# jfdev001/algebraic-multigrid

Measured on AMD Instinct MI355X. Metric: V-cycles/sec, 2D Poisson N=4096^2 (fine-grid smoother HBM GB/s under roofline), higher is better.
Workload: dtype f64; 1 GPU; 2D 5-point Poisson 4096x4096 (Grid::laplacian/rhs), true Jacobi smoother omega=0.6 2+2 sweeps, 16-level V-cycle, coarsest 511 dofs, fp64, 1xMI355X; smoother has no counterpart in the reference: pinned to the oracle twin; n=4096, dim=2, levels=16, smoother=jacobi, sweeps=2, graph=True, coarse_solve=band-chain (LDS-resident scalar recurrence, half-bandwidth <= 3, bit-exact), layout=dict

## Files before the change

algebraic-multigrid_amd/csrc/kernels.hip:

```cpp
#include <hip/hip_runtime.h>
#include <cstdlib>
#include <stdint.h>

#include <cstdio>
#include <type_traits>
#include <utility>
#include <vector>
#include <algorithm>
#include <cmath>

#include "kernels.hpp"

namespace amg_hip {

__device__ __forceinline__ void lds_barrier() {
  asm volatile("s_waitcnt lgkmcnt(0)\n\ts_barrier" ::: "memory");
}

constexpr bool mode_cheb(int m) { return (m & ~3) == 16; }
constexpr bool mode_jac(int m) { return m == CSR_JACOBI || mode_cheb(m); }
constexpr bool cheb_first(int m) { return (m & 1) != 0; }
constexpr bool cheb_last(int m) { return (m & 2) != 0; }
template <int MODE>
__device__ __forceinline__ double cheb_update(double t, double xi, double di, double alpha, double beta,
// ... 4612 lines not shown
                     omega, C, ring - 1);
  return hipGetLastError();
}
hipError_t launch_gs_scan(int64_t n, const DictRef& D, const double* b, double* u, double* s_old,
                          bool backward, int mode, double omega, int C, int ring, hipStream_t st) {
  if (n <= 0) return hipSuccess;
  if (!dict_args_ok(n, D.words, D.wmax, D.ntab) || C < 1 || C > GS_SCAN_MAX_CHUNK || ring < 2 || ring > 16384 ||
      (ring & (ring - 1)) || !s_old)
    return hipErrorInvalidValue;
  hipError_t r = hipSuccess;
  (void)dict_dispatch_wu(D.words, D.wmax, [&](auto W, auto U) {
    r = launch_gs_scan_wu<decltype(W)::value, decltype(U)::value>(n, D, b, u, s_old, backward ? 1 : 0,
                                                                  mode, omega, C, ring, st);
  });
  return r;
}

__device__ __forceinline__ bool spin_until_one(uint32_t* w, uint32_t* timeout) {
  const unsigned long long t0 = wall_clock64();
  while (__hip_atomic_load(w, __ATOMIC_ACQUIRE, __HIP_MEMORY_SCOPE_SYSTEM) != 1u) {
    if (wall_clock64() - t0 > 200000000ull) {
      __hip_atomic_store(timeout, 1u, __ATOMIC_RELAXED, __HIP_MEMORY_SCOPE_SYSTEM);
      return false;
    }
    __builtin_amdgcn_s_sleep(8);
  }
  __hip_atomic_store(w, 0u, __ATOMIC_RELAXED, __HIP_MEMORY_SCOPE_SYSTEM);
  return true;
}

__global__ __launch_bounds__(256) void halo_exchange_kernel(HaloArgs a) {
  const int t = threadIdx.x;
  if (t == 0) {
    if (a.cnt_prev > 0) spin_until_one(a.my_free_from_prev, a.timeout);
    if (a.cnt_next > 0) spin_until_one(a.my_free_from_next, a.timeout);
  }
  __syncthreads();
  for (int64_t i = t; i < a.cnt_prev; i += 256)
    __builtin_nontemporal_store(a.src_prev[i], a.dst_prev + i);
  for (int64_t i = t; i < a.cnt_next; i += 256)
    __builtin_nontemporal_store(a.src_next[i], a.dst_next + i);
  __threadfence_system();
  __syncthreads();
  if (t == 0) {
    if (a.cnt_prev > 0)
      __hip_atomic_store(a.data_at_prev, 1u, __ATOMIC_RELEASE, __HIP_MEMORY_SCOPE_SYSTEM);
    if (a.cnt_next > 0)
      __hip_atomic_store(a.data_at_next, 1u, __ATOMIC_RELEASE, __HIP_MEMORY_SCOPE_SYSTEM);
    if (a.recv_prev) spin_until_one(a.my_data_from_prev, a.timeout);
    if (a.recv_next) spin_until_one(a.my_data_from_next, a.timeout);
    __threadfence_system();
  }
}
__global__ void halo_ack_kernel(uint32_t* free_at_prev, uint32_t* free_at_next) {
  if (threadIdx.x == 0) {
    if (free_at_prev) __hip_atomic_store(free_at_prev, 1u, __ATOMIC_RELEASE, __HIP_MEMORY_SCOPE_SYSTEM);
    if (free_at_next) __hip_atomic_store(free_at_next, 1u, __ATOMIC_RELEASE, __HIP_MEMORY_SCOPE_SYSTEM);
  }
}
__global__ void halo_wait_free_kernel(HaloArgs a) {
  if (threadIdx.x == 0) {
    if (a.cnt_prev > 0) spin_until_one(a.my_free_from_prev, a.timeout);
    if (a.cnt_next > 0) spin_until_one(a.my_free_from_next, a.timeout);
  }
}
__global__ __launch_bounds__(256) void halo_copy_kernel(HaloArgs a) {
  const int64_t t = (int64_t)blockIdx.x * 256 + threadIdx.x, nt = (int64_t)gridDim.x * 256;
  for (int64_t i = t; i < a.cnt_prev; i += nt) __builtin_nontemporal_store(a.src_prev[i], a.dst_prev + i);
  for (int64_t i = t; i < a.cnt_next; i += nt) __builtin_nontemporal_store(a.src_next[i], a.dst_next + i);
  __threadfence_system();
}
__global__ void halo_publish_wait_kernel(HaloArgs a) {
  if (threadIdx.x == 0) {
    if (a.cnt_prev > 0)
      __hip_atomic_store(a.data_at_prev, 1u, __ATOMIC_RELEASE, __HIP_MEMORY_SCOPE_SYSTEM);
    if (a.cnt_next > 0)
      __hip_atomic_store(a.data_at_next, 1u, __ATOMIC_RELEASE, __HIP_MEMORY_SCOPE_SYSTEM);
    if (a.recv_prev) spin_until_one(a.my_data_from_prev, a.timeout);
    if (a.recv_next) spin_until_one(a.my_data_from_next, a.timeout);
    __threadfence_system();
  }
}
hipError_t launch_halo_exchange(const HaloArgs& a, hipStream_t st) {
  const int64_t big = a.cnt_prev > a.cnt_next ? a.cnt_prev : a.cnt_next;
  if (big <= 16384) {
    hipLaunchKernelGGL(halo_exchange_kernel, dim3(1), dim3(256), 0, st, a);
  } else {
    int64_t g = (big + 2047) / 2048;
    if (g > 256) g = 256;
    hipLaunchKernelGGL(halo_wait_free_kernel, dim3(1), dim3(64), 0, st, a);
    hipLaunchKernelGGL(halo_copy_kernel, dim3((unsigned)g), dim3(256), 0, st, a);
    hipLaunchKernelGGL(halo_publish_wait_kernel, dim3(1), dim3(64), 0, st, a);
  }
  return hipGetLastError();
}
hipError_t launch_halo_ack(uint32_t* free_at_prev, uint32_t* free_at_next, hipStream_t st) {
  if (!free_at_prev && !free_at_next) return hipSuccess;
  hipLaunchKernelGGL(halo_ack_kernel, dim3(1), dim3(64), 0, st, free_at_prev, free_at_next);
  return hipGetLastError();
}

__global__ void gather_wait_free_kernel(GatherArgs a) {
  const int g = threadIdx.x;
  if (g < a.world && g != a.rank) spin_until_one(a.my_free_from + g, a.timeout);
}
__global__ __launch_bounds__(256) void gather_copy_kernel(GatherArgs a) {
  const int g = blockIdx.y;
  double* dst = a.dst[g] + a.off;
  for (int64_t i = (int64_t)blockIdx.x * 256 + threadIdx.x; i < a.cnt; i += (int64_t)gridDim.x * 256)
    dst[i] = a.src[i];
  __threadfence_system();
}
__global__ void gather_publish_wait_kernel(GatherArgs a) {
  const int g = threadIdx.x;
  if (g < a.world && g != a.rank) {
    __hip_atomic_store(a.data_at[g], 1u, __ATOMIC_RELEASE, __HIP_MEMORY_SCOPE_SYSTEM);
    spin_until_one(a.my_data_from + g, a.timeout);
    __threadfence_system();
  }
}
__global__ void gather_ack_kernel(GatherArgs a) {
  const int g = threadIdx.x;
  if (g < a.world && g != a.rank)
    __hip_atomic_store(a.free_at[g], 1u, __ATOMIC_RELEASE, __HIP_MEMORY_SCOPE_SYSTEM);
}
hipError_t launch_gather(const GatherArgs& a, hipStream_t st) {
  hipLaunchKernelGGL(gather_wait_free_kernel, dim3(1), dim3(64), 0, st, a);
  int64_t gx = (a.cnt + 255) / 256;
  if (gx > 64) gx = 64;
  if (gx < 1) gx = 1;
  hipLaunchKernelGGL(gather_copy_kernel, dim3((unsigned)gx, (unsigned)a.world), dim3(256), 0, st, a);
  hipLaunchKernelGGL(gather_publish_wait_kernel, dim3(1), dim3(64), 0, st, a);
  return hipGetLastError();
}
hipError_t launch_gather_ack(const GatherArgs& a, hipStream_t st) {
  hipLaunchKernelGGL(gather_ack_kernel, dim3(1), dim3(64), 0, st, a);
  return hipGetLastError();
}

__device__ __forceinline__ double readlane_f64(double v, int lane) {
  const int lo = __builtin_amdgcn_readlane(__double2loint(v), lane);
  const int hi = __builtin_amdgcn_readlane(__double2hiint(v), lane);
  return __hiloint2double(hi, lo);
}
template <int LANE>
__device__ __forceinline__ void writelane_f64(double& dst, double uniform_v) {
  int lo = __double2loint(dst), hi = __double2hiint(dst);
  const int ulo = __builtin_amdgcn_readfirstlane(__double2loint(uniform_v));
  const int uhi = __builtin_amdgcn_readfirstlane(__double2hiint(uniform_v));
  asm volatile("v_writelane_b32 %0, %2, %4\n\tv_writelane_b32 %1, %3, %4"
               : "+v"(lo), "+v"(hi)
               : "s"(ulo), "s"(uhi), "n"(LANE));
  dst = __hiloint2double(hi, lo);
}

constexpr int BAND_CH = 32;

struct BandChunk {
  double lc[BAND_CH];
  double nx;
};

template <int M, bool FWD>
__device__ __forceinline__ void band_load(BandChunk& c, int64_t s0, int64_t n, int lane,
                                          const double* __restrict__ sched,
                                          const double* __restrict__ rhs) {
  if (lane < M) {
    const double* p = sched + s0 * M + lane;
#pragma unroll
    for (int i = 0; i < BAND_CH; ++i) c.lc[i] = p[i * M];
  } else {
#pragma unroll
    for (int i = 0; i < BAND_CH; ++i) c.lc[i] = 0.0;
  }
  const int64_t s2 = s0 + lane + M;
  const bool ok = lane < BAND_CH && s2 < n;
  const double v = rhs[ok ? (FWD ? s2 : n - 1 - s2) : 0];
  c.nx = ok ? v : 0.0;
}

template <int M, int PH, int I>
__device__ __forceinline__ void band_step(const BandChunk& c, double& acc, double& done) {
  constexpr int owner = (PH * BAND_CH + I) & (M - 1);
  const double vk = readlane_f64(acc, owner);
  acc -= c.lc[I] * vk;
  writelane_f64<I>(done, vk);
  writelane_f64<owner>(acc, readlane_f64(c.nx, I));
}
template <int M, int PH, int... I>
__device__ __forceinline__ void band_step_seq(const BandChunk& c, double& acc, double& done,
                                              std::integer_sequence<int, I...>) {
  (band_step<M, PH, I>(c, acc, done), ...);
}
template <int M, bool FWD, int PH>
__device__ __forceinline__ void band_steps(const BandChunk& c, double& acc, int64_t s0,
                                           int64_t n, int lane, double* __restrict__ x) {
  double done = 0.0;
  band_step_seq<M, PH>(c, acc, done, std::make_integer_sequence<int, BAND_CH>{});
  const int64_t s = s0 + lane;
  if (lane < BAND_CH && s < n) x[FWD ? s : n - 1 - s] = done;
}

template <int M, bool FWD>
__device__ __forceinline__ void band_pass(int64_t n, int lane, const double* __restrict__ sched,
                                          const double* __restrict__ rhs, double* __restrict__ x) {
  double acc = 0.0;
  if (lane < M && lane < n) acc = FWD ? rhs[lane] : rhs[n - 1 - lane];
  BandChunk A, B;
  band_load<M, FWD>(A, 0, n, lane, sched, rhs);
  for (int64_t s0 = 0; s0 < n; s0 += 2 * BAND_CH) {
    band_load<M, FWD>(B, s0 + BAND_CH, n, lane, sched, rhs);
    band_steps<M, FWD, 0>(A, acc, s0, n, lane, x);
    band_load<M, FWD>(A, s0 + 2 * BAND_CH, n, lane, sched, rhs);
    band_steps<M, FWD, 1>(B, acc, s0 + BAND_CH, n, lane, x);
  }
}

template <int M>
__global__ __launch_bounds__(64) void band_solve_kernel(
    int64_t n, const double* __restrict__ sched_f, const double* __restrict__ sched_b,
    const double* __restrict__ dg, const double* __restrict__ f, double* __restrict__ y,
    double* __restrict__ x, int64_t cstride) {
  const int lane = threadIdx.x;
  const int64_t co = (int64_t)blockIdx.x * cstride;
  f += co;
  y += co;
  x += co;
  band_pass<M, true>(n, lane, sched_f, f, y);
  __threadfence_block();
  for (int64_t i = lane; i < n; i += 64) y[i] = y[i] / dg[i];
  __threadfence_block();
  band_pass<M, false>(n, lane, sched_b, y, x);
}

constexpr int CHAIN_CH = 8;
__host__ __device__ inline int band_chain_pad(int n) { return (n + 2 * CHAIN_CH - 1) / (2 * CHAIN_CH) * (2 * CHAIN_CH) + 2 * CHAIN_CH; }
template <int W>
struct ChainChunk {
  double o[CHAIN_CH][W], r[CHAIN_CH];
};
template <int W>
__device__ __forceinline__ void band_chain_fetch(ChainChunk<W>& c, const double* op, const double* rv) {
#pragma unroll
  for (int i = 0; i < CHAIN_CH; ++i) {
#pragma unroll
    for (int t = 0; t < W; ++t) c.o[i][t] = op[i * W + t];
    c.r[i] = rv[i];
  }
}
template <int W>
__device__ __forceinline__ void band_chain_steps(const ChainChunk<W>& c, const ChainChunk<W>& nxt,
                                                 double (&prev)[W], double& early, int lane, double* out) {
  double res[CHAIN_CH];
#pragma unroll
  for (int i = 0; i < CHAIN_CH; ++i) {
    const double m = c.o[i][W - 1] * prev[W - 1];
    __builtin_amdgcn_sched_barrier(0);
    const double* on = i + 1 < CHAIN_CH ? c.o[i + 1] : nxt.o[0];
    double pr[W > 1 ? W - 1 : 1];
#pragma unroll
    for (int t = 0; t + 1 < W; ++t) pr[t] = on[t] * prev[t + 1];
    __builtin_amdgcn_sched_barrier(0);
    const double acc = early - m;
    __builtin_amdgcn_sched_barrier(0);
    double en = i + 1 < CHAIN_CH ? c.r[i + 1] : nxt.r[0];
#pragma unroll
    for (int t = 0; t + 1 < W; ++t) en -= pr[t];
    __builtin_amdgcn_sched_barrier(0);
#pragma unroll
    for (int t = 0; t + 1 < W; ++t) prev[t] = prev[t + 1];
    prev[W - 1] = acc;
    res[i] = acc;
    early = en;
  }
  if (lane == 0) {
#pragma unroll
    for (int i = 0; i < CHAIN_CH; ++i) out[i] = res[i];
  }
}
template <int W>
__device__ __forceinline__ void band_chain_pass(int n, const double* ops, double* v) {
  const int lane = threadIdx.x;
  double prev[W];
#pragma unroll
  for (int t = 0; t < W; ++t) prev[t] = 0.0;
  ChainChunk<W> A, B;
  band_chain_fetch<W>(A, ops, v);
  double early = A.r[0];
#pragma unroll
  for (int t = 0; t + 1 < W; ++t) early -= A.o[0][t] * prev[t];
  for (int s0 = 0; s0 < n; s0 += 2 * CHAIN_CH) {
    const double* op = ops + s0 * W;
    double* rv = v + s0;
    band_chain_fetch<W>(B, op + CHAIN_CH * W, rv + CHAIN_CH);
    __builtin_amdgcn_sched_barrier(0);
    band_chain_steps<W>(A, B, prev, early, lane, rv);
    __builtin_amdgcn_sched_barrier(0);
    band_chain_fetch<W>(A, op + 2 * CHAIN_CH * W, rv + 2 * CHAIN_CH);
    __builtin_amdgcn_sched_barrier(0);
    band_chain_steps<W>(B, A, prev, early, lane, rv + CHAIN_CH);
    __builtin_amdgcn_sched_barrier(0);
  }
}
__device__ __forceinline__ void band_chain_stage(const double* __restrict__ src, double* dst, int valid,
                                                 int total, int lane) {
  constexpr int R = 16;
  for (int base = 0; base < total; base += 64 * R) {
    double t[R];
#pragma unroll
    for (int j = 0; j < R; ++j) {
      const int k = base + j * 64 + lane;
      t[j] = k < valid ? src[k] : 0.0;
    }
#pragma unroll
    for (int j = 0; j < R; ++j) {
      const int k = base + j * 64 + lane;
      if (k < total) dst[k] = t[j];
    }
  }
}
template <int W>
__global__ __launch_bounds__(64) void band_chain_kernel(
    int n, const double* __restrict__ cf, const double* __restrict__ cb,
    const double* __restrict__ dg, const double* __restrict__ f, double* __restrict__ x, int n_h,
    const double* uh_in, double* uh_out, int pre, int64_t cstride) {
  extern __shared__ double chain_lds[];
  f += (int64_t)blockIdx.x * cstride;
  x += (int64_t)blockIdx.x * cstride;
  const int np = band_chain_pad(n);
  double* ops = chain_lds;
  double* v = chain_lds + np * W;
  double* opb = pre ? v + np : ops;
  const int lane = threadIdx.x;
  double dgv[32];
#pragma unroll
  for (int q = 0; q < 32; ++q) {
    const int s = lane + 64 * q;
    dgv[q] = s < n ? dg[n - 1 - s] : 1.0;
  }
  double a0[8], a1[8];
  auto fetch_fine = [&](int j0) {
#pragma unroll
    for (int q = 0; q < 8; ++q) {
      const int i = 2 * (j0 + q * 64 + lane);
      a0[q] = i < n_h ? uh_in[i] : 0.0;
      a1[q] = i + 1 < n_h ? uh_in[i + 1] : 0.0;
    }
  };
  if (uh_out) fetch_fine(0);
  band_chain_stage(cf, ops, n * W, np * W, lane);
  band_chain_stage(f, v, n, np, lane);
  if (pre) band_chain_stage(cb, opb, n * W, np * W, lane);
  lds_barrier();
  band_chain_pass<W>(n, ops, v);
  lds_barrier();
  double z[32];
#pragma unroll
  for (int q = 0; q < 32; ++q) {
    const int s = lane + 64 * q;
    z[q] = s < n ? v[n - 1 - s] / dgv[q] : 0.0;
  }
  if (!pre) band_chain_stage(cb, opb, n * W, n * W, lane);
  lds_barrier();
#pragma unroll
  for (int q = 0; q < 32; ++q) {
    const int s = lane + 64 * q;
    if (s < n) v[s] = z[q];
  }
  lds_barrier();
  band_chain_pass<W>(n, opb, v);
  lds_barrier();
  for (int s = lane; s < n; s += 64) x[n - 1 - s] = v[s];
  if (uh_out) {
    for (int j0 = 0; 2 * j0 < n_h; j0 += 64 * 8) {
      if (j0 > 0) fetch_fine(j0);
#pragma unroll
      for (int q = 0; q < 8; ++q) {
        const int j = j0 + q * 64 + lane, i = 2 * j;
        if (i >= n_h) continue;
        double t0 = 0.0, t1 = 0.0;
        const double b = (j < n) ? v[n - 1 - j] : 0.0;
        if (j >= 1 && j - 1 < n) t0 += 0.5 * v[n - j];
        if (j < n) {
          t0 += 0.5 * b;
          t1 += 1.0 * b;
        }
        uh_out[i] = a0[q] + t0;
        if (i + 1 < n_h) uh_out[i + 1] = a1[q] + t1;
      }
    }
  }
}
bool band_chain_ok(int64_t n, int64_t w) { return w >= 1 && w <= 3 && n >= 1 && n <= 2048; }
hipError_t launch_band_chain(int64_t n, int w, const double* cf, const double* cb, const double* dg,
                             const double* f, double* x, hipStream_t st, int64_t n_h, const double* uh_in,
                             double* uh_out, int cols, int64_t cstride) {
  if (!band_chain_ok(n, w) || (uh_out && (!uh_in || n_h < 1 || n_h > 2 * n + 2))) return hipErrorInvalidValue;
  if (cols < 1 || (uh_out && cols != 1)) return hipErrorInvalidValue;
  const size_t np = (size_t)band_chain_pad((int)n);
  const int pre = sizeof(double) * np * (size_t)(2 * w + 1) <= (size_t)48 * 1024 ? 1 : 0;
  const size_t lds = sizeof(double) * np * (size_t)(pre ? 2 * w + 1 : w + 1);
  switch (w) {
    case 1: hipLaunchKernelGGL(band_chain_kernel<1>, dim3(cols), dim3(64), lds, st, (int)n, cf, cb, dg, f, x, (int)n_h, uh_in, uh_out, pre, cstride); break;
    case 2: hipLaunchKernelGGL(band_chain_kernel<2>, dim3(cols), dim3(64), lds, st, (int)n, cf, cb, dg, f, x, (int)n_h, uh_in, uh_out, pre, cstride); break;
    default: hipLaunchKernelGGL(band_chain_kernel<3>, dim3(cols), dim3(64), lds, st, (int)n, cf, cb, dg, f, x, (int)n_h, uh_in, uh_out, pre, cstride); break;
  }
  return hipGetLastError();
}

constexpr int TAIL_MAX_LEVELS = TAIL_LEVELS_MAX;
constexpr int TAIL_MAX_COARSE = 1024;
constexpr int TAIL_LDS_DOUBLES = 18432;
typedef TailLevelRef TailLevel;
typedef TailRef TailArgs;
int tail_max_coarse() { return TAIL_MAX_COARSE; }
__host__ __device__ inline int tail_pad(int n) { return (n + 3) & ~1; }
__host__ __device__ inline size_t tail_lds_doubles(const TailArgs& A) {
  size_t d = 0;
  int nmax = 0;
  for (int q = 0; q < A.nlev; ++q) {
    d += 2 * (size_t)tail_pad(A.L[q].n) + 1024 + 1024 + 512 + (size_t)((A.L[q].n + 15) / 16) * 2;
    nmax = A.L[q].n > nmax ? A.L[q].n : nmax;
  }
  d += 2 * (size_t)tail_pad(nmax) + (size_t)tail_pad(A.nc) + (size_t)band_chain_pad(A.nc) * (size_t)(A.wc + 1);
  return d;
}
struct TailLds {
  int U, F, tabJ, tabR, wtab, rt;
};
template <int MODE>
__device__ __forceinline__ void tail_rows(int n, const DictEntry* tab, const uint64_t* wtab, const uint8_t* rt,
                                          const double* x, const double* f, double* out, double omega) {
  for (int row0 = (int)threadIdx.x * 2; row0 < n; row0 += 2048) {
    DictStream<2, 2> s;
    dict_fetch<MODE, 2, false, 2>(s, row0, n, nullptr, rt, f, x, 0);
    dict_expand<2, 2>(s, wtab);
    double res[2];
    dict_rows<MODE, 2, 9, 2>(s, row0, tab, x, omega, 0, res);
    if (s.live[0]) out[row0] = res[0];
    if (s.live[1]) out[row0 + 1] = res[1];
  }
}
__device__ __forceinline__ void tail_prolong(int n_h, int n_H, const double* uH, const double* base, double* out) {
  for (int j = threadIdx.x; 2 * j < n_h; j += 1024) {
    const int i = 2 * j;
    double t0 = 0.0, t1 = 0.0;
    const double b = (j < n_H) ? uH[j] : 0.0;
    if (j >= 1 && j - 1 < n_H) t0 += 0.5 * uH[j - 1];
    if (j < n_H) {
      t0 += 0.5 * b;
      t1 += 1.0 * b;
    }
    out[i] = base[i] + t0;
    if (i + 1 < n_h) out[i + 1] = base[i + 1] + t1;
  }
}
template <int W>
__global__ __launch_bounds__(1024) void tail_kernel(TailArgs A) {
  __shared__ __attribute__((aligned(16))) double tail_lds[TAIL_LDS_DOUBLES];
  TailLds P[TAIL_MAX_LEVELS];
  int p = 0, nmax = 0;
  for (int q = 0; q < A.nlev; ++q) {
    const int n = A.L[q].n, np = tail_pad(n);
    P[q].U = p; p += np;
    P[q].F = p; p += np;
    P[q].tabJ = p; p += 1024;
    P[q].tabR = p; p += 1024;
    P[q].wtab = p; p += 512;
    P[q].rt = p; p += ((n + 15) / 16) * 2;
    nmax = n > nmax ? n : nmax;
  }
  double* const T = tail_lds + p; p += tail_pad(nmax);
  double* const R = tail_lds + p; p += tail_pad(nmax);
  const int Uc = p; p += tail_pad(A.nc);
  const int npc = band_chain_pad(A.nc);
  double* const ops = tail_lds + p;
  const int voff = p + npc * W;
  double* const v = tail_lds + voff;
  if (voff + npc > TAIL_LDS_DOUBLES) return;
  const double omega = A.omega;
  const int tid = (int)threadIdx.x;
#define TAIL_D(off) (tail_lds + (off))
#define TAIL_TAB(off) reinterpret_cast<DictEntry*>(tail_lds + (off))
#define TAIL_W(off) reinterpret_cast<uint64_t*>(tail_lds + (off))
#define TAIL_B(off) reinterpret_cast<uint8_t*>(tail_lds + (off))
  for (int q = 0; q < A.nlev; ++q) {
    const TailLevel& L = A.L[q];
    if (tid < 256) {
      const int t = tid;
      const double val = t < L.ntab ? L.dval[t] : 0.0;
      const int32_t o = t < L.ntab ? L.doff[t] : 0;
      DictEntry e;
      e.a = o == 0 ? 0.0 : val;
      e.d = (o == 0 && t < L.ntab) ? val : 0.0;
      e.off8 = o * 8;
      e.pad[0] = e.pad[1] = e.pad[2] = 0;
      TAIL_TAB(P[q].tabJ)[t] = e;
      e.a = val;
      e.d = 0.0;
      TAIL_TAB(P[q].tabR)[t] = e;
      TAIL_W(P[q].wtab)[2 * t] = L.rwords[(size_t)t * L.words];
      TAIL_W(P[q].wtab)[2 * t + 1] = L.words == 2 ? L.rwords[(size_t)t * 2 + 1] : ~(uint64_t)0;
    }
    for (int r = tid; r < ((L.n + 15) / 16) * 16; r += 1024) TAIL_B(P[q].rt)[r] = r < L.n ? L.rtype[r] : (uint8_t)255;
  }
  for (int r = tid; r < tail_pad(A.L[0].n); r += 1024) {
    TAIL_D(P[0].F)[r] = r < A.L[0].n ? A.L[0].f[r] : 0.0;
    T[r] = r < A.L[0].n ? A.L[0].tmp[r] : 0.0;
  }
  for (int k = tid; k < npc * W; k += 1024) ops[k] = k < A.nc * W ? A.cf[k] : 0.0;
  __syncthreads();
  for (int li = 0; li < A.nlev; ++li) {
    const int n = A.L[li].n;
    const bool last = li + 1 == A.nlev;
    const int nH = last ? A.nc : A.L[li + 1].n;
    const double* dH = last ? A.diagc : A.L[li + 1].diag;
    const TailLds Q = P[li];
    tail_rows<CSR_JACOBI>(n, TAIL_TAB(Q.tabJ), TAIL_W(Q.wtab), TAIL_B(Q.rt), T, TAIL_D(Q.F), TAIL_D(Q.U),
                          omega);
    __syncthreads();
    tail_rows<CSR_RESID>(n, TAIL_TAB(Q.tabR), TAIL_W(Q.wtab), TAIL_B(Q.rt), TAIL_D(Q.U), TAIL_D(Q.F), R,
                         omega);
    if (tid < 2) R[n + tid] = 0.0;
    __syncthreads();
    double* FH = TAIL_D(last ? voff : P[li + 1 < A.nlev ? li + 1 : li].F);
    for (int j = tid; j < nH; j += 1024) {
      const int i = 2 * j;
      double sum = 0.0;
      if (i < n) sum += 0.5 * R[i];
      if (i + 1 < n) sum += 1.0 * R[i + 1];
      if (i + 2 < n) sum += 0.5 * R[i + 2];
      FH[j] = sum;
      const double xi = 0.0, acc = 0.0;
      const double d = dH[j];
      T[j] = (d == 0.0) ? xi : xi + omega * ((sum - acc) / d - xi);
    }
    if (last)
      for (int j = nH + tid; j < npc; j += 1024) v[j] = 0.0;
    __syncthreads();
  }
  {
    const int n = A.nc;
    if (tid >= 64)
      for (int j = tid - 64; j < n; j += 960) {
        A.fc[j] = v[j];
        A.tmpc[j] = T[j];
      }
    __syncthreads();
    if (tid < 64) band_chain_pass<W>(n, ops, v);
    __syncthreads();
    double z = 0.0;
    if (tid < n) z = v[n - 1 - tid] / A.dg[n - 1 - tid];
    for (int k = tid; k < n * W; k += 1024) ops[k] = A.cb[k];
    __syncthreads();
    if (tid < n) v[tid] = z;
    __syncthreads();
    if (tid < 64) band_chain_pass<W>(n, ops, v);
    __syncthreads();
    if (tid < n) {
      const double x = v[tid];
      TAIL_D(Uc)[n - 1 - tid] = x;
      A.uc[n - 1 - tid] = x;
    }
    __syncthreads();
  }
  int uH = Uc;
  int nH = A.nc;
  for (int li = A.nlev - 1; li >= 0; --li) {
    const int n = A.L[li].n;
    const TailLds Q = P[li];
    tail_prolong(n, nH, TAIL_D(uH), TAIL_D(Q.U), T);
    __syncthreads();
    tail_rows<CSR_JACOBI>(n, TAIL_TAB(Q.tabJ), TAIL_W(Q.wtab), TAIL_B(Q.rt), T, TAIL_D(Q.F), R, omega);
    __syncthreads();
    tail_rows<CSR_JACOBI>(n, TAIL_TAB(Q.tabJ), TAIL_W(Q.wtab), TAIL_B(Q.rt), R, TAIL_D(Q.F), TAIL_D(Q.U), omega);
    __syncthreads();
    uH = Q.U;
    nH = n;
  }
  tail_prolong(A.n_fine, nH, TAIL_D(uH), A.uf_in, A.uf_out);
  for (int li = 0; li < A.nlev; ++li) {
    const TailLevel& L = A.L[li];
    for (int r = tid; r < L.n; r += 1024) {
      L.u[r] = TAIL_D(P[li].U)[r];
      if (li > 0) const_cast<double*>(L.f)[r] = TAIL_D(P[li].F)[r];
    }
  }
#undef TAIL_D
#undef TAIL_TAB
#undef TAIL_W
#undef TAIL_B
}
bool tail_level_ok(int64_t n, const DictRef& D, int hb) {
  return D.rtype && D.rwords && !D.nt && hb >= 0 && n >= 256 && n <= 4095 && D.wmax <= 9 && D.words >= 1 &&
         D.words <= 2 && D.ntab <= 255;
}
size_t tail_lds_bytes(const TailRef& A) { return sizeof(double) * tail_lds_doubles(A); }
size_t tail_lds_capacity() { return sizeof(double) * (size_t)TAIL_LDS_DOUBLES; }
hipError_t launch_tail(const TailArgs& A, hipStream_t st) {
  if (A.nlev < 1 || A.nlev > TAIL_MAX_LEVELS || A.nc < 1 || A.nc > TAIL_MAX_COARSE || !band_chain_ok(A.nc, A.wc) ||
      tail_lds_bytes(A) > tail_lds_capacity() || A.n_fine < 1 || !A.uf_in || !A.uf_out)
    return hipErrorInvalidValue;
  for (int q = 0; q < A.nlev; ++q)
    if (A.L[q].n < 2 || !A.L[q].rtype || !A.L[q].rwords || !A.L[q].doff || !A.L[q].dval || !A.L[q].f || !A.L[q].u ||
        !A.L[q].tmp || !A.L[q].diag || A.L[q].ntab < 1 || A.L[q].ntab > 255)
      return hipErrorInvalidValue;
  switch (A.wc) {
    case 1: hipLaunchKernelGGL(tail_kernel<1>, dim3(1), dim3(1024), 0, st, A); break;
    case 2: hipLaunchKernelGGL(tail_kernel<2>, dim3(1), dim3(1024), 0, st, A); break;
    default: hipLaunchKernelGGL(tail_kernel<3>, dim3(1), dim3(1024), 0, st, A); break;
  }
  return hipGetLastError();
}

template <bool FWD>
__device__ __forceinline__ void band_wide_pass(int64_t n, int w, int ringmask, double* ring,
                                               const double* __restrict__ sched,
                                               const double* rhs, double* out) {
  const int lane = threadIdx.x;
  const int64_t nb = (n + 63) / 64;
  const int64_t stride = (int64_t)(w + 64) * 64;
  for (int k = lane; k <= ringmask; k += 64) ring[k] = 0.0;
  __syncthreads();
  for (int64_t b = 0; b < nb; ++b) {
    const int64_t r0 = b * 64, i = r0 + lane;
    const bool live = i < n;
    double acc = live ? rhs[FWD ? i : n - 1 - i] : 0.0;
    const double* __restrict__ Lp = sched + b * stride + lane;
    const int64_t tl = (int64_t)w - i;
    const int tlo = tl > 0 ? (int)tl : 0, thi = w - lane;
    if (b > 0) {
#pragma unroll 4
      for (int t = 0; t < w; ++t) {
        const double v = Lp[(int64_t)t * 64];
        const double yk = ring[(int)((i - w + t) & ringmask)];
        const double p = v * yk;
        acc = (t >= tlo && t < thi) ? acc - p : acc;
      }
    }
    const double* __restrict__ Ld = Lp + (int64_t)w * 64;
#pragma unroll 16
    for (int s = 0; s < 64; ++s) {
      const double vk = readlane_f64(acc, s);
      const double p = Ld[s * 64] * vk;
      acc = (lane > s) ? acc - p : acc;
    }
    if (live) {
      ring[(int)(i & ringmask)] = acc;
      out[FWD ? i : n - 1 - i] = acc;
    }
    __syncthreads();
  }
}
__global__ __launch_bounds__(64) void band_wide_kernel(
    int64_t n, int w, int ringmask, const double* __restrict__ sched_f,
    const double* __restrict__ sched_b, const double* __restrict__ dg, const double* f, double* y,
    double* x, int64_t cstride) {
  extern __shared__ double ring[];
  const int64_t co = (int64_t)blockIdx.x * cstride;
  f += co;
  y += co;
  x += co;
  band_wide_pass<true>(n, w, ringmask, ring, sched_f, f, y);
  __threadfence_block();
  for (int64_t i = threadIdx.x; i < n; i += 64) y[i] = y[i] / dg[i];
  __threadfence_block();
  __syncthreads();
  band_wide_pass<false>(n, w, ringmask, ring, sched_b, y, x);
}
hipError_t launch_band_wide(int64_t n, int64_t w, const double* sched_f, const double* sched_b,
                            const double* dg, const double* f, double* y, double* x,
                            hipStream_t st, int cols, int64_t cstride) {
  if (n <= 0) return hipSuccess;
  if (cols < 1) return hipErrorInvalidValue;
  int64_t R = 128;
  while (R < w + 64) R *= 2;
  if (R * 8 > 65536 || w < 1) return hipErrorInvalidValue;
  hipLaunchKernelGGL(band_wide_kernel, dim3(cols), dim3(64), (size_t)R * 8, st, n, (int)w, (int)(R - 1),
                     sched_f, sched_b, dg, f, y, x, cstride);
  return hipGetLastError();
}

template <int M, bool FWD>
__global__ __launch_bounds__(64) void spike_local_kernel(SpikeArgs a, const double* rhs,
                                                         double* out) {
  const int lane = threadIdx.x;
  const int64_t r0 = (int64_t)blockIdx.x * a.c;
  const int64_t nl = (a.n - r0 < a.c) ? a.n - r0 : a.c;
  band_pass<M, FWD>(nl, lane, (FWD ? a.sched_f : a.sched_b) + (int64_t)blockIdx.x * a.sched_stride,
                    rhs + r0, out + r0);
}
template <int M, bool FWD>
__global__ __launch_bounds__(64) void spike_boundary_kernel(SpikeArgs a, const double* g,
                                                            double* bnd) {
  const int k = threadIdx.x;
  const int w = a.w, wq = a.w > 0 ? a.w : 1;
  const bool act = k < w;
  const int kc = k < M ? k : 0;
  const double* blocks = FWD ? a.Vt : a.Wh;
  double cur[M], nxt[M];
#pragma unroll
  for (int j = 0; j < M; ++j) cur[j] = 0.0;
  double t = 0.0;
  for (int s = 0; s < a.P; ++s) {
    const int q = FWD ? s : a.P - 1 - s;
    const int64_t r0 = (int64_t)q * a.c;
    const int64_t nl = (a.n - r0 < a.c) ? a.n - r0 : a.c;
    const int64_t row = FWD ? r0 + nl - w + k : r0 + k;
// ... 2703 lines not shown
```

Measured before the change: 1571 V-cycles/s.

## Widen band-chain coarse solve block to 256 threads with prefetched operand staging

```diff
diff --git a/algebraic-multigrid_amd/csrc/kernels.hip b/algebraic-multigrid_amd/csrc/kernels.hip
--- a/algebraic-multigrid_amd/csrc/kernels.hip
+++ b/algebraic-multigrid_amd/csrc/kernels.hip
@@ -4938,25 +4938,37 @@
     __builtin_amdgcn_sched_barrier(0);
   }
 }
-__device__ __forceinline__ void band_chain_stage(const double* __restrict__ src, double* dst, int valid,
-                                                 int total, int lane) {
-  constexpr int R = 16;
-  for (int base = 0; base < total; base += 64 * R) {
+constexpr int CHAIN_T = 256;
+template <int R>
+__device__ __forceinline__ void band_chain_load(double (&t)[R], const double* __restrict__ src, int valid,
+                                                int base, int tid) {
+#pragma unroll
+  for (int j = 0; j < R; ++j) {
+    const int k = base + j * CHAIN_T + tid;
+    t[j] = src[min(k, valid - 1)];
+  }
+}
+template <int R>
+__device__ __forceinline__ void band_chain_store(const double (&t)[R], double* dst, int valid, int base,
+                                                 int tid) {
+#pragma unroll
+  for (int j = 0; j < R; ++j) {
+    const int k = base + j * CHAIN_T + tid;
+    if (k < valid) dst[k] = t[j];
+  }
+}
+template <int R>
+__device__ __forceinline__ void band_chain_stage_rest(const double* __restrict__ src, double* dst, int valid,
+                                                      int total, int tid) {
+  for (int base = CHAIN_T * R; base < valid; base += CHAIN_T * R) {
     double t[R];
-#pragma unroll
-    for (int j = 0; j < R; ++j) {
-      const int k = base + j * 64 + lane;
-      t[j] = k < valid ? src[k] : 0.0;
-    }
-#pragma unroll
-    for (int j = 0; j < R; ++j) {
-      const int k = base + j * 64 + lane;
-      if (k < total) dst[k] = t[j];
-    }
-  }
+    band_chain_load<R>(t, src, valid, base, tid);
+    band_chain_store<R>(t, dst, valid, base, tid);
+  }
+  for (int k = valid + tid; k < total; k += CHAIN_T) dst[k] = 0.0;
 }
 template <int W>
-__global__ __launch_bounds__(64) void band_chain_kernel(
+__global__ __launch_bounds__(CHAIN_T) void band_chain_kernel(
     int n, const double* __restrict__ cf, const double* __restrict__ cb,
     const double* __restrict__ dg, const double* __restrict__ f, double* __restrict__ x, int n_h,
     const double* uh_in, double* uh_out, int pre, int64_t cstride) {
@@ -4967,63 +4979,84 @@
   double* ops = chain_lds;
   double* v = chain_lds + np * W;
   double* opb = pre ? v + np : ops;
-  const int lane = threadIdx.x;
-  double dgv[32];
-#pragma unroll
-  for (int q = 0; q < 32; ++q) {
-    const int s = lane + 64 * q;
-    dgv[q] = s < n ? dg[n - 1 - s] : 1.0;
-  }
-  double a0[8], a1[8];
+  const int tid = threadIdx.x;
+  constexpr int RO = 4, RF = 2;
+  const int nhalf = (n + 1) / 2;
+  double d_lo = dg[min(tid, n - 1)], d_hi = dg[max(n - 1 - tid, 0)];
+  double a0[2] = {0.0, 0.0}, a1[2] = {0.0, 0.0};
   auto fetch_fine = [&](int j0) {
 #pragma unroll
-    for (int q = 0; q < 8; ++q) {
-      const int i = 2 * (j0 + q * 64 + lane);
-      a0[q] = i < n_h ? uh_in[i] : 0.0;
-      a1[q] = i + 1 < n_h ? uh_in[i + 1] : 0.0;
+    for (int q = 0; q < 2; ++q) {
+      const int i = 2 * (j0 + q * CHAIN_T + tid);
+      a0[q] = uh_in[min(i, n_h - 1)];
+      a1[q] = uh_in[min(i + 1, n_h - 1)];
     }
   };
+  double tb[RO], tf[RF], to[RO];
+  band_chain_load<RO>(tb, cb, n * W, 0, tid);
+  band_chain_load<RF>(tf, f, n, 0, tid);
+  band_chain_load<RO>(to, cf, n * W, 0, tid);
   if (uh_out) fetch_fine(0);
-  band_chain_stage(cf, ops, n * W, np * W, lane);
-  band_chain_stage(f, v, n, np, lane);
-  if (pre) band_chain_stage(cb, opb, n * W, np * W, lane);
+  band_chain_store<RO>(to, ops, n * W, 0, tid);
+  band_chain_store<RF>(tf, v, n, 0, tid);
+  band_chain_stage_rest<RO>(cf, ops, n * W, np * W, tid);
+  band_chain_stage_rest<RF>(f, v, n, np, tid);
+  if (pre) {
+    band_chain_store<RO>(tb, opb, n * W, 0, tid);
+    band_chain_stage_rest<RO>(cb, opb, n * W, np * W, tid);
+  }
   lds_barrier();
-  band_chain_pass<W>(n, ops, v);
+  if (tid < 64) band_chain_pass<W>(n, ops, v);
   lds_barrier();
-  double z[32];
-#pragma unroll
-  for (int q = 0; q < 32; ++q) {
-    const int s = lane + 64 * q;
-    z[q] = s < n ? v[n - 1 - s] / dgv[q] : 0.0;
-  }
-  if (!pre) band_chain_stage(cb, opb, n * W, n * W, lane);
+  for (int i = tid; i < nhalf; i += CHAIN_T) {
+    const int m = n - 1 - i;
+    if (i >= CHAIN_T) {
+      d_lo = dg[i];
+      d_hi = dg[m];
+    }
+    const double z_lo = v[i] / d_lo, z_hi = v[m] / d_hi;
+    v[m] = z_lo;
+    v[i] = z_hi;
+  }
+  if (!pre) {
+    band_chain_store<RO>(tb, opb, n * W, 0, tid);
+    band_chain_stage_rest<RO>(cb, opb, n * W, n * W, tid);
+  }
   lds_barrier();
-#pragma unroll
-  for (int q = 0; q < 32; ++q) {
-    const int s = lane + 64 * q;
-    if (s < n) v[s] = z[q];
-  }
+  if (tid < 64) band_chain_pass<W>(n, opb, v);
   lds_barrier();
-  band_chain_pass<W>(n, opb, v);
-  lds_barrier();
-  for (int s = lane; s < n; s += 64) x[n - 1 - s] = v[s];
+  double o0[2], o1[2];
+  auto prolong_sums = [&](int j0) {
+#pragma unroll
+    for (int q = 0; q < 2; ++q) {
+      const int j = j0 + q * CHAIN_T + tid;
+      double t0 = 0.0, t1 = 0.0;
+      const double b = (j < n) ? v[n - 1 - j] : 0.0;
+      if (j >= 1 && j - 1 < n) t0 += 0.5 * v[n - j];
+      if (j < n) {
+        t0 += 0.5 * b;
+        t1 += 1.0 * b;
+      }
+      o0[q] = a0[q] + t0;
+      o1[q] = a1[q] + t1;
+    }
+  };
+  auto prolong_store = [&](int j0) {
+#pragma unroll
+    for (int q = 0; q < 2; ++q) {
+      const int i = 2 * (j0 + q * CHAIN_T + tid);
+      if (i < n_h) uh_out[i] = o0[q];
+      if (i + 1 < n_h) uh_out[i + 1] = o1[q];
+    }
+  };
+  prolong_sums(0);
+  for (int s = tid; s < n; s += CHAIN_T) x[n - 1 - s] = v[s];
   if (uh_out) {
-    for (int j0 = 0; 2 * j0 < n_h; j0 += 64 * 8) {
-      if (j0 > 0) fetch_fine(j0);
-#pragma unroll
-      for (int q = 0; q < 8; ++q) {
-        const int j = j0 + q * 64 + lane, i = 2 * j;
-        if (i >= n_h) continue;
-        double t0 = 0.0, t1 = 0.0;
-        const double b = (j < n) ? v[n - 1 - j] : 0.0;
-        if (j >= 1 && j - 1 < n) t0 += 0.5 * v[n - j];
-        if (j < n) {
-          t0 += 0.5 * b;
-          t1 += 1.0 * b;
-        }
-        uh_out[i] = a0[q] + t0;
-        if (i + 1 < n_h) uh_out[i + 1] = a1[q] + t1;
-      }
+    prolong_store(0);
+    for (int j0 = CHAIN_T * 2; 2 * j0 < n_h; j0 += CHAIN_T * 2) {
+      fetch_fine(j0);
+      prolong_sums(j0);
+      prolong_store(j0);
     }
   }
 }
@@ -5037,9 +5070,9 @@
   const int pre = sizeof(double) * np * (size_t)(2 * w + 1) <= (size_t)48 * 1024 ? 1 : 0;
   const size_t lds = sizeof(double) * np * (size_t)(pre ? 2 * w + 1 : w + 1);
   switch (w) {
-    case 1: hipLaunchKernelGGL(band_chain_kernel<1>, dim3(cols), dim3(64), lds, st, (int)n, cf, cb, dg, f, x, (int)n_h, uh_in, uh_out, pre, cstride); break;
-    case 2: hipLaunchKernelGGL(band_chain_kernel<2>, dim3(cols), dim3(64), lds, st, (int)n, cf, cb, dg, f, x, (int)n_h, uh_in, uh_out, pre, cstride); break;
-    default: hipLaunchKernelGGL(band_chain_kernel<3>, dim3(cols), dim3(64), lds, st, (int)n, cf, cb, dg, f, x, (int)n_h, uh_in, uh_out, pre, cstride); break;
+    case 1: hipLaunchKernelGGL(band_chain_kernel<1>, dim3(cols), dim3(CHAIN_T), lds, st, (int)n, cf, cb, dg, f, x, (int)n_h, uh_in, uh_out, pre, cstride); break;
+    case 2: hipLaunchKernelGGL(band_chain_kernel<2>, dim3(cols), dim3(CHAIN_T), lds, st, (int)n, cf, cb, dg, f, x, (int)n_h, uh_in, uh_out, pre, cstride); break;
+    default: hipLaunchKernelGGL(band_chain_kernel<3>, dim3(cols), dim3(CHAIN_T), lds, st, (int)n, cf, cb, dg, f, x, (int)n_h, uh_in, uh_out, pre, cstride); break;
   }
   return hipGetLastError();
 }
```

After: 1591 V-cycles/s, median of 6. 1.3% higher.
